# SKA-INAF/caesar-mrcnn

Measured on AMD Instinct MI355X. Metric: train images/sec (whole node) + detect ms/image, ResNet-101 256x256, higher is better.
Workload: dtype f32; 1 GPU; resnet101+FPN 256x256 3-class (+bg), nimg_per_gpu=4, train step (fwd+bwd+SGD), 512 train ROIs, 2000 proposals; global_batch=4, parallelism=dp1, weights=random init (Keras defaults)

## Files before the change

caesar-mrcnn_amd/_hip.py:

```python
import ctypes as C
import os
import threading

PKG_DIR = os.path.dirname(os.path.abspath(__file__))
LIB_PATH = os.path.join(PKG_DIR, "libmrcnn_hip.so")


class HipPathError(RuntimeError):
    pass


class ConvDesc(C.Structure):
    _fields_ = [(n, C.c_int32) for n in (
        "N", "H", "W", "Cin", "Cout", "KH", "KW", "stride", "pad_t", "pad_l", "OH", "OW",
        "act", "res_mode", "out_mode", "cmod")] + [
        ("out_n_stride", C.c_int64), ("out_h_stride", C.c_int64), ("out_w_stride", C.c_int64)]


class ConvProblem(C.Structure):
    _fields_ = [("d", ConvDesc)] + [(n, C.c_void_p) for n in ("x", "w", "bias", "scale", "shift", "res", "out", "z_out")]


class WgradProblem(C.Structure):
    _fields_ = [("d", ConvDesc), ("x", C.c_void_p), ("dy", C.c_void_p), ("dw", C.c_void_p), ("accumulate", C.c_int32)]
# ... 120 lines not shown
    "mrcnn_conv2d_fwd_h16_res": (C.c_int, [C.POINTER(ConvDesc), C.c_int] + [_P] * 9),
    "mrcnn_conv2d_fwd_h16_supported": (C.c_int, [C.POINTER(ConvDesc), C.c_int]),
    "mrcnn_conv2d_dgrad_ep_h16": (C.c_int, [C.POINTER(ConvDesc), C.c_int, _P, _P, _P, _P, C.POINTER(BwdEpilogueH16), _P]),
    "mrcnn_conv2d_dgrad_ep": (C.c_int, [C.POINTER(ConvDesc), _P, _P, _P, _P, C.POINTER(BwdEpilogue), _P, C.c_size_t, _P]),
    "mrcnn_conv2d_wgrad_h16_workspace": (C.c_size_t, [C.POINTER(ConvDesc)]),
    "mrcnn_conv2d_wgrad_h16": (C.c_int, [C.POINTER(ConvDesc), C.c_int, _P, _P, _P, _P, C.c_size_t, C.c_int, C.c_float, _P]),
    "mrcnn_mask_out_fwd_h16": (C.c_int, [C.c_int, _P, _P, _P, _P, C.c_int64, C.c_int, C.c_int, _P]),
    "mrcnn_mask_out_bwd_h16": (C.c_int, [C.c_int] + [_P] * 8 + [C.c_int64, C.c_int, C.c_int, C.c_int, C.c_int, C.c_float, _P]),
    "mrcnn_weights_to_h16": (C.c_int, [_P, _P, _P, C.c_int, C.c_int, C.c_int, C.c_int, C.c_int, _P]),
    "mrcnn_weights_to_h16_batched": (C.c_int, [_P, _P, C.c_int, C.c_int, C.c_int, _P]),
    "mrcnn_cast_to_h16": (C.c_int, [_P, _P, C.c_int64, C.c_int, C.c_float, _P]),
    "mrcnn_epilogue_bwd_h16": (C.c_int, [C.c_int] + [_P] * 10 + [C.c_int64, C.c_int, C.c_int, C.c_float, _P]),
    "mrcnn_epilogue_bwd_h16_dy": (C.c_int, [C.c_int] + [_P] * 11 + [C.c_int64, C.c_int, C.c_int, C.c_float, _P]),
    "mrcnn_cast_from_h16": (C.c_int, [_P, _P, C.c_int64, C.c_int, C.c_float, _P]),
    "mrcnn_axpy_from_h16": (C.c_int, [_P, _P, C.c_int64, C.c_int, C.c_float, _P]),
    "mrcnn_rpn_targets_workspace": (C.c_size_t, [C.POINTER(RpnTargetDesc)]),
    "mrcnn_rpn_targets": (C.c_int, [C.POINTER(RpnTargetDesc)] + [_P] * 7 + [C.c_size_t, _P]),
    "mrcnn_detection_workspace": (C.c_size_t, [C.POINTER(DetectionDesc)]),
    "mrcnn_detection_fwd": (C.c_int, [C.POINTER(DetectionDesc)] + [_P] * 6 + [C.c_size_t, _P]),
    "mrcnn_losses_workspace": (C.c_size_t, [C.POINTER(LossDesc)]),
    "mrcnn_losses_fwd_bwd": (C.c_int, [C.POINTER(LossDesc)] + [_P] * 18 + [C.c_size_t, _P]),
    "mrcnn_grad_prepare": (C.c_int, [_P, _P, C.c_float, _P, C.c_int64, _P, _P]),
    "mrcnn_sumsq": (C.c_int, [_P, C.c_int64, _P, _P]),
    "mrcnn_sgd_momentum": (C.c_int, [_P, _P, _P, _P, C.c_float, C.c_float, C.c_float, _P, C.c_int64, _P]),
    "mrcnn_sgd_momentum_guarded": (C.c_int, [_P, _P, _P, _P, C.c_float, C.c_float, C.c_float, _P, C.c_int64, _P, _P]),
    "mrcnn_winograd_buffer_floats": (C.c_size_t, [C.c_int, C.c_int, C.c_int, C.c_int, C.c_int]),
    "mrcnn_winograd_weights": (C.c_int, [_P, _P, C.c_int, C.c_int, C.c_int, _P]),
    "mrcnn_gemm_batched_f32": (C.c_int, [_P, _P, _P, C.c_int, C.c_int, C.c_int, C.c_int, _P]),
    "mrcnn_winograd_gemm": (C.c_int, [_P, _P, _P, C.c_int, C.c_int, C.c_int, C.c_int, _P]),
    "mrcnn_winograd_group_floats": (C.c_size_t, [C.POINTER(WinoGroup), C.c_int, C.c_int]),
    "mrcnn_winograd_input_g": (C.c_int, [_P, _P, C.c_int, C.c_int, C.c_int, C.c_int, C.POINTER(WinoGroup), _P]),
    "mrcnn_winograd_weights_g": (C.c_int, [_P, _P, C.c_int, C.c_int, C.c_int, C.c_int, _P]),
    "mrcnn_winograd_output_g": (C.c_int, [_P, _P, _P, _P, _P, _P, C.c_int, C.c_int, C.c_int, C.c_int, C.c_int, C.POINTER(WinoGroup), _P]),
    "mrcnn_winograd_output_bwd_g": (C.c_int, [_P, _P, _P, _P, _P, _P, _P, _P, _P, _P, C.c_int, C.c_int, C.c_int, C.c_int, C.c_int,
                                             C.POINTER(WinoGroup), _P]),
    "mrcnn_winograd_output_bwd_zmask_g": (C.c_int, [_P] * 10 + [C.c_int, C.c_int, C.c_int, C.c_int, C.POINTER(WinoGroup), _P]),
    "mrcnn_winograd_dy_g": (C.c_int, [_P, _P, C.c_int, C.c_int, C.c_int, C.c_int, C.POINTER(WinoGroup), _P]),
    "mrcnn_winograd_dw_g": (C.c_int, [_P, _P, C.c_int, C.c_int, C.c_int, C.c_int, C.c_int, _P]),
    "mrcnn_deconv2x2_gemm": (C.c_int, [_P, _P, _P, _P, C.c_int, C.c_int, C.c_int, C.c_int, C.c_int, C.c_int, _P]),
    "mrcnn_allreduce_load": (C.c_int, [C.c_char_p]),
    "mrcnn_allreduce_unique_id": (C.c_int, [_P]),
    "mrcnn_allreduce_init": (C.c_int, [C.POINTER(_P), _P, C.c_int, C.c_int]),
    "mrcnn_allreduce_scratch": (C.c_size_t, [C.c_int, C.c_int64, C.c_int]),
    "mrcnn_allreduce_grad": (C.c_int, [_P, _P, C.c_int64, C.c_int64, C.c_int, _P, C.c_size_t, _P]),
    "mrcnn_allreduce_direct_plan": (C.c_int, [C.c_int, C.c_int, C.c_int64, C.c_int64, C.c_int, _P, _P, _P, _P]),
    "mrcnn_allreduce_direct_simulate": (C.c_int, [_P, _P, C.c_size_t, C.c_int, C.c_int64, C.c_int64, _P]),
    "mrcnn_allreduce_destroy": (C.c_int, [_P]),
    "mrcnn_allreduce_last_error": (C.c_char_p, []),
    "mrcnn_tuning_set": (C.c_int, [C.c_char_p, C.c_longlong]),
    "mrcnn_hip_version": (C.c_char_p, []),
}

_lib = None
_proxy = None
_tape = None
_tape_owner = None

_NO_RECORD = ("_workspace", "_tiles_check", "_outline_check", "_draw_check", "_supported", "_status_offset", "_version", "mrcnn_allreduce_", "_scratch", "_floats")


class _LibProxy(object):

    def __init__(self, real):
        self._real = real

    def __getattr__(self, name):
        real = getattr(self._real, name)
        if any(k in name for k in _NO_RECORD):
            f = real
        else:
            def f(*args, _real=real):
                rc = _real(*args)
                t = _tape
                if t is not None and not rc and _tape_owner == threading.get_ident():
                    t.append((_real, args))
                return rc
        setattr(self, name, f)
        return f


def tape_begin():
    global _tape, _tape_owner
    assert _tape is None, "a launch tape is already being recorded"
    _tape, _tape_owner = [], threading.get_ident()
    return _tape


def tape_end():
    global _tape, _tape_owner
    t, _tape, _tape_owner = _tape, None, None
    return t
# ... 83 lines not shown
```

caesar-mrcnn_amd/csrc/winograd.hip:

```cpp
#include "common.h"
#include <type_traits>
#include <string.h>

template <int CV> struct WinoVec;
template <> struct WinoVec<4> { typedef f32x4 type; };
template <> struct WinoVec<2> { typedef float type __attribute__((ext_vector_type(2))); };

template <int OT, typename V> __device__ __forceinline__ void wino_bt(const V (&d)[OT + 2], V (&t)[OT + 2]) {
    if constexpr (OT == 2) {
        t[0] = d[0] - d[2];
        t[1] = d[1] + d[2];
        t[2] = d[2] - d[1];
        t[3] = d[1] - d[3];
    } else {
        const V a = d[4] - 4.f * d[2], b = d[3] - 4.f * d[1], c = d[4] - d[2], e = 2.f * (d[3] - d[1]);
        t[0] = 4.f * d[0] - 5.f * d[2] + d[4];
        t[1] = a + b;
        t[2] = a - b;
        t[3] = c + e;
        t[4] = c - e;
        t[5] = 4.f * d[1] - 5.f * d[3] + d[5];
    }
}
template <int OT, typename V> __device__ __forceinline__ void wino_at(const V (&m)[OT + 2], V (&y)[OT]) {
// ... 158 lines not shown
            vec zv, o;
#pragma unroll
            for (int e = 0; e < CV; ++e) {
                zv[e] = y[b][e] + bi[e];
                float v = sc[e] * zv[e] + sh[e];
                if (act == MRCNN_ACT_RELU) v = fmaxf(v, 0.f);
                o[e] = v;
            }
            if (z) *(vec*)(z + addr) = zv;
            *(vec*)(out + addr) = o;
        }
    }
}

template <int OTH, int OTW, int CV>
__global__ __launch_bounds__(256) void winograd_output_kernel(const float* __restrict__ Mt, float* __restrict__ out, float* __restrict__ z,
                                                              const float* __restrict__ bias, const float* __restrict__ scale,
                                                              const float* __restrict__ shift, int N, int H, int W, int C, long long T,
                                                              long long Tp, int act, const WinoGrp g) {
    typedef typename WinoVec<CV>::type vec;
    const int cn = C / CV;
    const long long i = (long long)blockIdx.x * 256 + threadIdx.x;
    if (i >= T * cn) return;
    const long long t = i / cn;
    const int c = (int)(i - t * cn) * CV;
    vec bi = {}, sc, sh = {};
#pragma unroll
    for (int e = 0; e < CV; ++e) sc[e] = 1.f;
    if (bias) bi = *(const vec*)(bias + c);
    if (scale) { sc = *(const vec*)(scale + c); sh = *(const vec*)(shift + c); }
    wino_output_tile<OTH, OTW, CV>(Mt, out, z, bi, sc, sh, H, W, C, Tp, act, g, t, c);
}

template <int OTH, int OTW, int CV>
__device__ __forceinline__ void wino_output_bwd_tile(const float* __restrict__ Mt, float* __restrict__ dz_out, const float* __restrict__ below_out,
                                                     const float* __restrict__ below_z, const typename WinoVec<CV>::type sc,
                                                     const typename WinoVec<CV>::type mu, const typename WinoVec<CV>::type rs,
                                                     const typename WinoVec<CV>::type fsh, bool zmask, bool want_dg, int H, int W, int C,
                                                     long long Tp, int act, const WinoGrp& g, long long t, int c,
                                                     typename WinoVec<CV>::type& a_db, typename WinoVec<CV>::type& a_dg,
                                                     typename WinoVec<CV>::type& a_bias) {
    typedef typename WinoVec<CV>::type vec;
    constexpr int ITH = OTH + 2, ITW = OTW + 2;
    const WinoTile q = wino_tile(t, g.th_n, g.tw_n);
    vec s[OTH][ITW];
#pragma unroll
    for (int k = 0; k < ITW; ++k) {
        vec col[ITH], o[OTH];
#pragma unroll
        for (int r = 0; r < ITH; ++r) col[r] = *(const vec*)(Mt + ((long long)(r * ITW + k) * Tp + t) * C + c);
        wino_at<OTH>(col, o);
#pragma unroll
        for (int a = 0; a < OTH; ++a) s[a][k] = o[a];
    }
#pragma unroll
    for (int a = 0; a < OTH; ++a) {
        vec y[OTW];
        wino_at<OTW>(s[a], y);
        const int oh = g.oh0 + OTH * q.th + a;
        if (oh >= H) continue;
#pragma unroll
        for (int b = 0; b < OTW; ++b) {
            const int ow = g.ow0 + OTW * q.tw + b;
            if (ow >= W) continue;
            const long long addr = (((long long)q.n * H + oh) * W + ow) * C + c;
            vec gg = y[b], dz, zz = {};
            if (want_dg || zmask) zz = *(const vec*)(below_z + addr);
            if (act == MRCNN_ACT_RELU) {
                if (zmask) {
#pragma unroll
                    for (int e = 0; e < CV; ++e) {
                        const float v = sc[e] * zz[e] + fsh[e];
                        gg[e] = v > 0.f ? gg[e] : 0.f;
                    }
                } else {
                    const vec oo = *(const vec*)(below_out + addr);
#pragma unroll
                    for (int e = 0; e < CV; ++e) gg[e] = oo[e] > 0.f ? gg[e] : 0.f;
                }
            }
#pragma unroll
            for (int e = 0; e < CV; ++e) dz[e] = gg[e] * sc[e];
            *(vec*)(dz_out + addr) = dz;
            if (want_dg) {
#pragma unroll
                for (int e = 0; e < CV; ++e) a_dg[e] += gg[e] * (zz[e] - mu[e]) * rs[e];
            }
#pragma unroll
            for (int e = 0; e < CV; ++e) { a_db[e] += gg[e]; a_bias[e] += dz[e]; }
        }
    }
}

template <int OTH, int OTW, int CV>
__global__ __launch_bounds__(256) void winograd_output_bwd_kernel(const float* __restrict__ Mt, float* __restrict__ dz_out,
                                                                  const float* __restrict__ below_out, const float* __restrict__ below_z,
                                                                  const float* __restrict__ scale, const float* __restrict__ mean,
                                                                  const float* __restrict__ rstd, float* dgamma, float* dbeta, float* dbias,
                                                                  int N, int H, int W, int C, long long T, long long Tp, int act,
                                                                  long long tiles_per_block, int lg, const WinoGrp g,
                                                                  const float* __restrict__ fwd_shift) {
    typedef typename WinoVec<CV>::type vec;
    constexpr int ITH = OTH + 2, ITW = OTW + 2;
    __shared__ float sacc[3 * 4 * 256];
    const int L = 1 << lg, R = 256 >> lg;
    for (int c = threadIdx.x; c < 3 * CV * L; c += 256) sacc[c] = 0.f;
    __syncthreads();
    const int rsub = threadIdx.x >> lg, lane = threadIdx.x & (L - 1);
    const int c = lane * CV;
    const long long t0 = (long long)blockIdx.x * tiles_per_block;
    long long t1 = t0 + tiles_per_block;
    if (t1 > T) t1 = T;
    vec sc, mu = {}, rs = {}, fsh = {};
#pragma unroll
    for (int e = 0; e < CV; ++e) sc[e] = 1.f;
    if (scale) sc = *(const vec*)(scale + c);
    if (dgamma) { mu = *(const vec*)(mean + c); rs = *(const vec*)(rstd + c); }
    const bool zmask = fwd_shift != nullptr;
    if (zmask) fsh = *(const vec*)(fwd_shift + c);
    vec a_db = {}, a_dg = {}, a_bias = {};
    for (long long t = t0 + rsub; t < t1; t += R)
        wino_output_bwd_tile<OTH, OTW, CV>(Mt, dz_out, below_out, below_z, sc, mu, rs, fsh, zmask, dgamma != nullptr, H, W, C, Tp, act, g, t, c,
                                           a_db, a_dg, a_bias);
#pragma unroll
    for (int k = 0; k < CV; ++k) {
        if (dbeta || dgamma) atomicAdd(&sacc[lane * CV + k], a_db[k]);
        if (dgamma) atomicAdd(&sacc[CV * L + lane * CV + k], a_dg[k]);
        if (dbias) atomicAdd(&sacc[2 * CV * L + lane * CV + k], a_bias[k]);
    }
    __syncthreads();
    for (int j = threadIdx.x; j < CV * L; j += 256) {
        if (dbeta) atomicAdd(&dbeta[j], sacc[j]);
        if (dgamma) atomicAdd(&dgamma[j], sacc[CV * L + j]);
        if (dbias) atomicAdd(&dbias[j], sacc[2 * CV * L + j]);
    }
}

template <int OTH, int OTW, int CV>
__global__ __launch_bounds__(256) void winograd_dy_kernel(const float* __restrict__ dy, float* __restrict__ dM, int N, int H, int W, int C,
                                                          long long T, long long Tp, const WinoGrp g) {
    typedef typename WinoVec<CV>::type vec;
    constexpr int ITH = OTH + 2, ITW = OTW + 2;
    const int cn = C / CV;
    const long long i = (long long)blockIdx.x * 256 + threadIdx.x;
    if (i >= T * cn) return;
    const long long t = i / cn;
    const int c = (int)(i - t * cn) * CV;
    const WinoTile q = wino_tile(t, g.th_n, g.tw_n);
    vec u[ITH][OTW];
#pragma unroll
    for (int b = 0; b < OTW; ++b) {
        vec col[OTH], o[ITH];
#pragma unroll
        for (int a = 0; a < OTH; ++a) {
            const int oh = g.oh0 + OTH * q.th + a, ow = g.ow0 + OTW * q.tw + b;
            vec val = {};
            if (oh < H && ow < W) val = *(const vec*)(dy + (((long long)q.n * H + oh) * W + ow) * C + c);
            col[a] = val;
        }
        wino_a<OTH>(col, o);
#pragma unroll
        for (int r = 0; r < ITH; ++r) u[r][b] = o[r];
    }
#pragma unroll
    for (int r = 0; r < ITH; ++r) {
        vec m[ITW];
        wino_a<OTW>(u[r], m);
// ... 211 lines not shown

extern "C" size_t mrcnn_winograd_group_floats(const mrcnn_wino_group* g, int N, int C) {
    if (!g || N <= 0 || C <= 0 || (g->oth != 2 && g->oth != 4) || (g->otw != 2 && g->otw != 4) || g->th_n <= 0 || g->tw_n <= 0) return 0;
    return (size_t)wino_grp_nb(g) * (size_t)wino_rows(wino_grp_tiles(g, N)) * (size_t)C;
}

extern "C" int mrcnn_winograd_input_g(const float* x, float* V, int N, int H, int W, int C, const mrcnn_wino_group* g, void* stream) {
    if (!x || !V || !wino_grp_ok(g, N, H, W, C)) return MRCNN_ERR_ARG;
    const long long T = wino_grp_tiles(g, N);
    const WinoGrp k = {g->th_n, g->tw_n, g->oh0, g->ow0};
    const dim3 g4((unsigned)cdiv64(T * C / 4, 256)), g2((unsigned)cdiv64(T * C / 2, 256));
    WINO_LAUNCH_G(winograd_input_kernel, g, g4, g2, x, V, N, H, W, C, T, wino_rows(T), k);
    return mrcnn_launch_status();
}

extern "C" int mrcnn_winograd_weights_g(const float* w, float* U, int Cin, int Cout, int oth, int otw, void* stream) {
    if (!w || !U || Cin <= 0 || Cout <= 0 || (oth != 2 && oth != 4) || (otw != 2 && otw != 4)) return MRCNN_ERR_ARG;
    const dim3 grid((unsigned)cdiv64((long long)Cin * Cout, 256));
    WINO_LAUNCH_W(winograd_weight_kernel, oth, otw, grid, w, U, Cin, Cout);
    return mrcnn_launch_status();
}

extern "C" int mrcnn_winograd_output_g(const float* Mt, float* out, float* z, const float* bias, const float* scale, const float* shift,
                                       int N, int H, int W, int C, int act, const mrcnn_wino_group* g, void* stream) {
    if (!Mt || !out || !wino_grp_ok(g, N, H, W, C) || (scale && !shift)) return MRCNN_ERR_ARG;
    if (act != MRCNN_ACT_NONE && act != MRCNN_ACT_RELU) return MRCNN_ERR_UNSUPPORTED;
    const long long T = wino_grp_tiles(g, N);
    const WinoGrp k = {g->th_n, g->tw_n, g->oh0, g->ow0};
    const dim3 g4((unsigned)cdiv64(T * C / 4, 256)), g2((unsigned)cdiv64(T * C / 2, 256));
    WINO_LAUNCH_G(winograd_output_kernel, g, g4, g2, Mt, out, z, bias, scale, shift, N, H, W, C, T, wino_rows(T), act, k);
    return mrcnn_launch_status();
}

static int wino_output_bwd_g(const float* Mt, float* dz_below, const float* below_out, const float* below_z, const float* scale,
                             const float* mean, const float* rstd, float* dgamma, float* dbeta, float* dbias, int N, int H,
                             int W, int C, int act, const mrcnn_wino_group* g, void* stream, const float* fwd_shift);

extern "C" int mrcnn_winograd_output_bwd_g(const float* Mt, float* dz_below, const float* below_out, const float* below_z, const float* scale,
                                           const float* mean, const float* rstd, float* dgamma, float* dbeta, float* dbias, int N, int H,
                                           int W, int C, int act, const mrcnn_wino_group* g, void* stream) {
    return wino_output_bwd_g(Mt, dz_below, below_out, below_z, scale, mean, rstd, dgamma, dbeta, dbias, N, H, W, C, act, g, stream, nullptr);
}

extern "C" int mrcnn_winograd_output_bwd_zmask_g(const float* Mt, float* dz_below, const float* below_z, const float* scale,
                                                 const float* shift, const float* mean, const float* rstd, float* dgamma, float* dbeta,
                                                 float* dbias, int N, int H, int W, int C, const mrcnn_wino_group* g, void* stream) {
    if (!below_z || !scale || !shift) return MRCNN_ERR_ARG;
    return wino_output_bwd_g(Mt, dz_below, nullptr, below_z, scale, mean, rstd, dgamma, dbeta, dbias, N, H, W, C, MRCNN_ACT_RELU, g, stream, shift);
}

static int wino_output_bwd_g(const float* Mt, float* dz_below, const float* below_out, const float* below_z, const float* scale,
                             const float* mean, const float* rstd, float* dgamma, float* dbeta, float* dbias, int N, int H,
                             int W, int C, int act, const mrcnn_wino_group* g, void* stream, const float* fwd_shift) {
    if (!Mt || !dz_below || !wino_grp_ok(g, N, H, W, C)) return MRCNN_ERR_ARG;
    if ((act != MRCNN_ACT_NONE && act != MRCNN_ACT_RELU) || (act == MRCNN_ACT_RELU && !below_out && !fwd_shift)) return MRCNN_ERR_ARG;
    if (dgamma && (!below_z || !mean || !rstd)) return MRCNN_ERR_ARG;
    const int cv = wino_grp_cv(g);
    const int cn = C / cv;
    if (cn > 256 || (cn & (cn - 1))) return MRCNN_ERR_UNSUPPORTED;
    int lg = 0;
    while ((1 << lg) < cn) ++lg;
    const long long T = wino_grp_tiles(g, N);
    const long long R = 256 >> lg;
    long long per = (T + 2047) / 2048;
    per = (per + R - 1) / R * R;
    const dim3 grid((unsigned)cdiv64(T, per));
    const WinoGrp k = {g->th_n, g->tw_n, g->oh0, g->ow0};
    WINO_LAUNCH_G(winograd_output_bwd_kernel, g, grid, grid, Mt, dz_below, below_out, below_z, scale, mean, rstd, dgamma, dbeta, dbias, N, H, W,
                  C, T, wino_rows(T), act, per, lg, k, fwd_shift);
    return mrcnn_launch_status();
}

extern "C" int mrcnn_winograd_dy_g(const float* dy, float* dM, int N, int H, int W, int C, const mrcnn_wino_group* g, void* stream) {
    if (!dy || !dM || !wino_grp_ok(g, N, H, W, C)) return MRCNN_ERR_ARG;
    const long long T = wino_grp_tiles(g, N);
    const WinoGrp k = {g->th_n, g->tw_n, g->oh0, g->ow0};
    const dim3 g4((unsigned)cdiv64(T * C / 4, 256)), g2((unsigned)cdiv64(T * C / 2, 256));
    WINO_LAUNCH_G(winograd_dy_kernel, g, g4, g2, dy, dM, N, H, W, C, T, wino_rows(T), k);
    return mrcnn_launch_status();
}

extern "C" int mrcnn_winograd_dw_g(const float* dU, float* dw_hwio, int Cin, int Cout, int accumulate, int oth, int otw, void* stream) {
    if (!dU || !dw_hwio || Cin <= 0 || Cout <= 0 || (oth != 2 && oth != 4) || (otw != 2 && otw != 4)) return MRCNN_ERR_ARG;
    const dim3 grid((unsigned)cdiv64((long long)Cin * Cout, 256));
    WINO_LAUNCH_W(winograd_dw_kernel, oth, otw, grid, dU, dw_hwio, Cin, Cout, accumulate);
    return mrcnn_launch_status();
}

extern "C" size_t mrcnn_winograd_buffer_floats(int N, int H, int W, int C, int tile) {
    if ((tile != 2 && tile != 4) || (tile == 2 && ((H & 1) || (W & 1)))) return 0;
    if (!(N > 0 && H > 0 && W > 0 && C > 0 && !(C & 3))) return 0;
    const mrcnn_wino_group g = {tile, tile, wino_tdim(H, tile), wino_tdim(W, tile), 0, 0};
    return mrcnn_winograd_group_floats(&g, N, C);
}

extern "C" int mrcnn_winograd_weights(const float* w, float* U, int Cin, int Cout, int tile, void* stream) {
    return mrcnn_winograd_weights_g(w, U, Cin, Cout, tile, tile, stream);
}

extern "C" int mrcnn_winograd_gemm(const float* V, const float* U, float* Mt, int nb, int rows, int K, int N, void* stream) {
    if (!V || !U || !Mt || nb <= 0 || rows <= 0 || rows % 128 || K <= 0 || K % 16 || N <= 0 || N % 128) return MRCNN_ERR_ARG;
    const long long M = (long long)nb * rows;
// ... 41 lines not shown
```

caesar-mrcnn_amd/ops.py:

```python
import ctypes as C
import math
import os

import torch

from . import _hip
from ._hip import (ACT_NONE, ACT_RELU, ACT_SIGMOID, OUT_DECONV2, OUT_NHWC, RES_NONE, RES_SAME, RES_UP2,
                   check, current_stream, ptr)

BN_EPS = 1e-3


def _need_cuda(*ts):
    for t in ts:
        if t is not None and not t.is_cuda:
            raise _hip.HipPathError("hot-path operators need device tensors (got a CPU tensor)")
        if t is not None and not t.is_contiguous():
            raise _hip.HipPathError("hot-path operators need contiguous tensors")


def same_padding(size, k, stride):
    out = -(-size // stride)
    total = max((out - 1) * stride + k - size, 0)
    return out, total // 2
# ... 1243 lines not shown


def winograd_v_floats(xshape, tile=None):
    N, H, W, Cin = xshape
    if tile is None:
        tile = winograd_tile(xshape)
    lib = _hip.lib()
    return sum(lib.mrcnn_winograd_group_floats(C.byref(g), N, Cin) for g in winograd_groups(H, W, tile))


def conv2d_winograd(x, U, bias=None, scale=None, shift=None, act=ACT_NONE, out=None, z_out=None, keep_v=None, after_input=None):
    _need_cuda(x, bias, scale, shift, out, z_out, keep_v)
    N, H, W, _ = x.shape
    cout = (U[0] if isinstance(U, (list, tuple)) else U).shape[2]
    if out is None:
        out = empty((N, H, W, cout), torch.float32, x.device)
    lib = _hip.lib()

    def finish(g, Mt):
        check(lib.mrcnn_winograd_output_g(ptr(Mt), ptr(out), ptr(z_out), ptr(bias), ptr(scale), ptr(shift), N, H, W, cout, act, C.byref(g),
                                          current_stream()), "mrcnn_winograd_output_g")

    _winograd_run(x, U, finish, keep_v, after_input)
    return out


def conv2d_dgrad_ep_winograd(dz, Ut, below_out, below_z, scale, mean, rstd, dgamma, dbeta, dbias, act, fwd_shift=None):
    _need_cuda(dz, below_out, below_z, scale, mean, rstd, dgamma, dbeta, dbias, fwd_shift)
    N, H, W, _ = dz.shape
    cout = (Ut[0] if isinstance(Ut, (list, tuple)) else Ut).shape[2]
    out = empty((N, H, W, cout), torch.float32, dz.device)
    lib = _hip.lib()
    zmask = act == ACT_RELU and fwd_shift is not None and below_z is not None and scale is not None

    def finish(g, Mt):
        if zmask:
            check(lib.mrcnn_winograd_output_bwd_zmask_g(ptr(Mt), ptr(out), ptr(below_z), ptr(scale), ptr(fwd_shift), ptr(mean), ptr(rstd),
                                                        ptr(dgamma), ptr(dbeta), ptr(dbias), N, H, W, cout, C.byref(g), current_stream()),
                  "mrcnn_winograd_output_bwd_zmask_g")
            return
        check(lib.mrcnn_winograd_output_bwd_g(ptr(Mt), ptr(out), ptr(below_out), ptr(below_z), ptr(scale), ptr(mean), ptr(rstd),
                                              ptr(dgamma), ptr(dbeta), ptr(dbias), N, H, W, cout, act, C.byref(g), current_stream()),
              "mrcnn_winograd_output_bwd_g")

    _winograd_run(dz, Ut, finish)
    return out


def conv2d_wgrad_winograd(V, xshape, dz, dw, accumulate=False, tile=None):
    _need_cuda(V, dz, dw)
    N, H, W, Cin = xshape
    cout = dz.shape[3]
    if tile is None:
        tile = winograd_tile(xshape)
    groups = winograd_groups(H, W, tile)
    lib = _hip.lib()
    nvs = [lib.mrcnn_winograd_group_floats(C.byref(g), N, Cin) for g in groups]
    nms = [lib.mrcnn_winograd_group_floats(C.byref(g), N, cout) for g in groups]
    assert V.numel() == sum(nvs), "V was made with another tiling"
    dM_all = workspace(max(nms) * 4, dz.device, "winograd_dm")
    dU_all = workspace(36 * Cin * cout * 4, dz.device, "winograd_du")
    off = 0
    for gi, g in enumerate(groups):
        nb = _wino_nb(g)
        rows = nms[gi] // (nb * cout)
        T = N * g.th_n * g.tw_n
        dM = dM_all[:nms[gi] * 4].view(torch.float32).view(nb, rows, cout)
        dU = dU_all[:nb * Cin * cout * 4].view(torch.float32).view(nb, Cin, cout)
        check(lib.mrcnn_winograd_dy_g(ptr(dz), ptr(dM), N, H, W, cout, C.byref(g), current_stream()), "mrcnn_winograd_dy_g")
        Vv = V[off:off + nvs[gi]].view(nb, rows, Cin)
        off += nvs[gi]
        items = [(Vv[k, :T].view(T, 1, 1, Cin), dM[k, :T].view(T, 1, 1, cout), (1, 1, Cin, cout), 1, "valid", dU[k].view(1, 1, Cin, cout), False)
                 for k in range(nb)]
        per = 16 if nb == 16 else 12
        for i in range(0, nb, per):
            if not conv2d_wgrad_multi(items[i:i + per]):
                for x_, dy_, wshape, stride, padding, dw_, acc in items[i:i + per]:
                    conv2d_wgrad(x_, dy_, wshape, stride, padding, dw=dw_, accumulate=acc)
# ... 150 lines not shown
```

include/mrcnn_hip.h:

```cpp
#ifndef MRCNN_HIP_H
#define MRCNN_HIP_H

#include <stddef.h>
#include <stdint.h>

#ifdef __cplusplus
extern "C" {
#endif

#define MRCNN_OK 0
#define MRCNN_ERR_ARG (-1)
#define MRCNN_ERR_LAUNCH (-2)
#define MRCNN_ERR_WORKSPACE (-3)
#define MRCNN_ERR_UNSUPPORTED (-4)

#define MRCNN_ACT_NONE 0
#define MRCNN_ACT_RELU 1
#define MRCNN_ACT_SIGMOID 2

#define MRCNN_RES_NONE 0
#define MRCNN_RES_SAME 1
#define MRCNN_RES_UP2 2

#define MRCNN_OUT_NHWC 0
// ... 293 lines not shown
int mrcnn_losses_fwd_bwd(const mrcnn_loss_desc* d, const int32_t* rpn_match, const float* rpn_bbox_t,
                         const float* rpn_class_logits, const float* rpn_bbox,
                         const int32_t* target_class_ids, const float* target_bbox,
                         const float* target_mask, const int32_t* active_class_ids,
                         const float* mrcnn_class_logits, const float* mrcnn_bbox,
                         const float* mrcnn_mask, float* losses, float* d_rpn_class_logits,
                         float* d_rpn_bbox, float* d_mrcnn_class_logits, float* d_mrcnn_bbox,
                         float* d_mrcnn_mask, void* workspace, size_t workspace_bytes, void* stream);

int mrcnn_grad_prepare(float* grads, const float* params, float grad_scale, const float* gran_coef,
                       int64_t n, float* sumsq_out, void* stream);
int mrcnn_sumsq(const float* g, int64_t n, float* out_scalar, void* stream);
int mrcnn_sgd_momentum(float* params, float* momentum_buf, const float* grads, const float* sumsq,
                       float clipnorm, float lr, float momentum, const float* gran_coef, int64_t n,
                       void* stream);
int mrcnn_sgd_momentum_guarded(float* params, float* momentum_buf, const float* grads, const float* sumsq,
                               float clipnorm, float lr, float momentum, const float* gran_coef, int64_t n,
                               unsigned* skipped_steps, void* stream);

typedef struct mrcnn_wino_group {
    int oth, otw;
    int th_n, tw_n;
    int oh0, ow0;
} mrcnn_wino_group;
size_t mrcnn_winograd_group_floats(const mrcnn_wino_group* g, int N, int C);
size_t mrcnn_winograd_buffer_floats(int N, int H, int W, int C, int tile);
int mrcnn_winograd_weights(const float* w_hwio, float* U, int Cin, int Cout, int tile, void* stream);
int mrcnn_winograd_weights_g(const float* w_hwio, float* U, int Cin, int Cout, int oth, int otw, void* stream);
int mrcnn_winograd_input_g(const float* x, float* V, int N, int H, int W, int C, const mrcnn_wino_group* g, void* stream);
int mrcnn_gemm_batched_f32(const float* V, const float* U, float* Mt, int nb, int rows, int K, int Cout, void* stream);
int mrcnn_winograd_gemm(const float* V, const float* U, float* Mt, int nb, int rows, int K, int Cout, void* stream);
int mrcnn_winograd_output_g(const float* Mt, float* out, float* z_out, const float* bias, const float* scale, const float* shift,
                            int N, int H, int W, int C, int act, const mrcnn_wino_group* g, void* stream);
int mrcnn_winograd_output_bwd_g(const float* Mt, float* dz_below, const float* below_out, const float* below_z, const float* scale,
                                const float* mean, const float* rstd, float* dgamma, float* dbeta, float* dbias, int N, int H, int W,
                                int C, int act, const mrcnn_wino_group* g, void* stream);
int mrcnn_winograd_output_bwd_zmask_g(const float* Mt, float* dz_below, const float* below_z, const float* scale, const float* shift,
                                      const float* mean, const float* rstd, float* dgamma, float* dbeta, float* dbias, int N, int H,
                                      int W, int C, const mrcnn_wino_group* g, void* stream);
int mrcnn_winograd_dy_g(const float* dy, float* dM, int N, int H, int W, int C, const mrcnn_wino_group* g, void* stream);
int mrcnn_winograd_dw_g(const float* dU, float* dw_hwio, int Cin, int Cout, int accumulate, int oth, int otw, void* stream);

int mrcnn_deconv2x2_gemm(const float* x, const float* w_gemm, const float* bias, float* out, int N, int H, int W, int Cin, int Cd,
                         int act, void* stream);

#define MRCNN_UNIQUE_ID_BYTES 128
#define MRCNN_ALLREDUCE_RCCL 0
#define MRCNN_ALLREDUCE_DIRECT 1
int mrcnn_allreduce_load(const char* librccl_path);
int mrcnn_allreduce_unique_id(void* id_128_bytes);
int mrcnn_allreduce_init(void** comm, const void* id_128_bytes, int rank, int world);
size_t mrcnn_allreduce_scratch(int world, int64_t max_range_floats, int algo);
int mrcnn_allreduce_grad(void* comm, float* grads, int64_t start, int64_t end, int algo, float* scratch,
                         size_t scratch_bytes, void* stream);
int mrcnn_allreduce_direct_plan(int world, int rank, int64_t start, int64_t end, int phase, int64_t* plan, int64_t* own_off,
                                int64_t* own_len, int64_t* slot_stride);
int mrcnn_allreduce_direct_simulate(float* const* grads, float* const* scratch, size_t scratch_bytes, int world, int64_t start,
                                    int64_t end, void* stream);
int mrcnn_allreduce_destroy(void* comm);
const char* mrcnn_allreduce_last_error(void);

int mrcnn_tuning_set(const char* key, long long value);

const char* mrcnn_hip_version(void);

#ifdef __cplusplus
}
#endif
#endif
```

Baseline: 111.7 images/s.

## Replace atomic reductions in Winograd output backward with per-block partials and sum kernel

The Winograd data-gradient output kernel now runs as a persistent grid capped at four blocks per CU. Each block writes per-channel partial sums for dbeta, dgamma and dbias to a workspace, and a separate kernel reduces them, replacing the shared and global atomics. The kernel also issues all Mt tile loads up front through buffer loads with 32-bit offsets, uses fast division for tile indexing, and is templated on the mask mode. This trades atomic contention and 64-bit address math for an extra kernel launch, a workspace, and higher register pressure from the preloaded tiles.

After: 113.1 images/s, median of 6. +1.3%, better.

```diff
diff --git a/caesar-mrcnn_amd/_hip.py b/caesar-mrcnn_amd/_hip.py
--- a/caesar-mrcnn_amd/_hip.py
+++ b/caesar-mrcnn_amd/_hip.py
@@ -176,9 +176,10 @@
     "mrcnn_winograd_input_g": (C.c_int, [_P, _P, C.c_int, C.c_int, C.c_int, C.c_int, C.POINTER(WinoGroup), _P]),
     "mrcnn_winograd_weights_g": (C.c_int, [_P, _P, C.c_int, C.c_int, C.c_int, C.c_int, _P]),
     "mrcnn_winograd_output_g": (C.c_int, [_P, _P, _P, _P, _P, _P, C.c_int, C.c_int, C.c_int, C.c_int, C.c_int, C.POINTER(WinoGroup), _P]),
-    "mrcnn_winograd_output_bwd_g": (C.c_int, [_P, _P, _P, _P, _P, _P, _P, _P, _P, _P, C.c_int, C.c_int, C.c_int, C.c_int, C.c_int,
-                                             C.POINTER(WinoGroup), _P]),
-    "mrcnn_winograd_output_bwd_zmask_g": (C.c_int, [_P] * 10 + [C.c_int, C.c_int, C.c_int, C.c_int, C.POINTER(WinoGroup), _P]),
+    "mrcnn_winograd_output_bwd_rows": (C.c_int, [C.POINTER(WinoGroup), C.c_int, C.c_int]),
+    "mrcnn_winograd_output_bwd_g": (C.c_int, [_P] * 8 + [C.c_int, C.c_int, C.c_int, C.c_int, C.c_int, C.POINTER(WinoGroup), _P]),
+    "mrcnn_winograd_output_bwd_zmask_g": (C.c_int, [_P] * 8 + [C.c_int, C.c_int, C.c_int, C.c_int, C.POINTER(WinoGroup), _P]),
+    "mrcnn_winograd_output_bwd_sums": (C.c_int, [_P, C.c_int, C.c_int, _P, _P, _P, _P]),
     "mrcnn_winograd_dy_g": (C.c_int, [_P, _P, C.c_int, C.c_int, C.c_int, C.c_int, C.POINTER(WinoGroup), _P]),
     "mrcnn_winograd_dw_g": (C.c_int, [_P, _P, C.c_int, C.c_int, C.c_int, C.c_int, C.c_int, _P]),
     "mrcnn_deconv2x2_gemm": (C.c_int, [_P, _P, _P, _P, C.c_int, C.c_int, C.c_int, C.c_int, C.c_int, C.c_int, _P]),
@@ -200,7 +201,7 @@
 _tape = None
 _tape_owner = None
 
-_NO_RECORD = ("_workspace", "_tiles_check", "_outline_check", "_draw_check", "_supported", "_status_offset", "_version", "mrcnn_allreduce_", "_scratch", "_floats")
+_NO_RECORD = ("_workspace", "_tiles_check", "_outline_check", "_draw_check", "_supported", "_status_offset", "_version", "mrcnn_allreduce_", "_scratch", "_floats", "_bwd_rows")
 
 
 class _LibProxy(object):
diff --git a/caesar-mrcnn_amd/csrc/winograd.hip b/caesar-mrcnn_amd/csrc/winograd.hip
--- a/caesar-mrcnn_amd/csrc/winograd.hip
+++ b/caesar-mrcnn_amd/csrc/winograd.hip
@@ -214,107 +214,157 @@
     wino_output_tile<OTH, OTW, CV>(Mt, out, z, bi, sc, sh, H, W, C, Tp, act, g, t, c);
 }
 
-template <int OTH, int OTW, int CV>
-__device__ __forceinline__ void wino_output_bwd_tile(const float* __restrict__ Mt, float* __restrict__ dz_out, const float* __restrict__ below_out,
-                                                     const float* __restrict__ below_z, const typename WinoVec<CV>::type sc,
-                                                     const typename WinoVec<CV>::type mu, const typename WinoVec<CV>::type rs,
-                                                     const typename WinoVec<CV>::type fsh, bool zmask, bool want_dg, int H, int W, int C,
-                                                     long long Tp, int act, const WinoGrp& g, long long t, int c,
-                                                     typename WinoVec<CV>::type& a_db, typename WinoVec<CV>::type& a_dg,
-                                                     typename WinoVec<CV>::type& a_bias) {
-    typedef typename WinoVec<CV>::type vec;
-    constexpr int ITH = OTH + 2, ITW = OTW + 2;
-    const WinoTile q = wino_tile(t, g.th_n, g.tw_n);
-    vec s[OTH][ITW];
-#pragma unroll
-    for (int k = 0; k < ITW; ++k) {
-        vec col[ITH], o[OTH];
-#pragma unroll
-        for (int r = 0; r < ITH; ++r) col[r] = *(const vec*)(Mt + ((long long)(r * ITW + k) * Tp + t) * C + c);
-        wino_at<OTH>(col, o);
-#pragma unroll
-        for (int a = 0; a < OTH; ++a) s[a][k] = o[a];
-    }
-#pragma unroll
-    for (int a = 0; a < OTH; ++a) {
-        vec y[OTW];
-        wino_at<OTW>(s[a], y);
-        const int oh = g.oh0 + OTH * q.th + a;
-        if (oh >= H) continue;
-#pragma unroll
-        for (int b = 0; b < OTW; ++b) {
-            const int ow = g.ow0 + OTW * q.tw + b;
-            if (ow >= W) continue;
-            const long long addr = (((long long)q.n * H + oh) * W + ow) * C + c;
-            vec gg = y[b], dz, zz = {};
-            if (want_dg || zmask) zz = *(const vec*)(below_z + addr);
-            if (act == MRCNN_ACT_RELU) {
-                if (zmask) {
-#pragma unroll
-                    for (int e = 0; e < CV; ++e) {
-                        const float v = sc[e] * zz[e] + fsh[e];
-                        gg[e] = v > 0.f ? gg[e] : 0.f;
-                    }
-                } else {
-                    const vec oo = *(const vec*)(below_out + addr);
-#pragma unroll
-                    for (int e = 0; e < CV; ++e) gg[e] = oo[e] > 0.f ? gg[e] : 0.f;
-                }
-            }
-#pragma unroll
-            for (int e = 0; e < CV; ++e) dz[e] = gg[e] * sc[e];
-            *(vec*)(dz_out + addr) = dz;
-            if (want_dg) {
-#pragma unroll
-                for (int e = 0; e < CV; ++e) a_dg[e] += gg[e] * (zz[e] - mu[e]) * rs[e];
-            }
-#pragma unroll
-            for (int e = 0; e < CV; ++e) { a_db[e] += gg[e]; a_bias[e] += dz[e]; }
-        }
-    }
-}
-
-template <int OTH, int OTW, int CV>
+template <int CV>
+__device__ __forceinline__ typename WinoVec<CV>::type wino_buffer_load(__amdgpu_buffer_rsrc_t rsrc, unsigned voff, unsigned soff) {
+    typename WinoVec<CV>::type r;
+    if constexpr (CV == 2) {
+        const auto v = __builtin_amdgcn_raw_buffer_load_b64(rsrc, (int)voff, (int)soff, 0);
+        r[0] = __uint_as_float(v[0]); r[1] = __uint_as_float(v[1]);
+    } else {
+        const auto v = __builtin_amdgcn_raw_buffer_load_b128(rsrc, (int)voff, (int)soff, 0);
+        r[0] = __uint_as_float(v[0]); r[1] = __uint_as_float(v[1]); r[2] = __uint_as_float(v[2]); r[3] = __uint_as_float(v[3]);
+    }
+    return r;
+}
+
+template <int OTH, int OTW, int CV, int MASK>
 __global__ __launch_bounds__(256) void winograd_output_bwd_kernel(const float* __restrict__ Mt, float* __restrict__ dz_out,
                                                                   const float* __restrict__ below_out, const float* __restrict__ below_z,
                                                                   const float* __restrict__ scale, const float* __restrict__ mean,
-                                                                  const float* __restrict__ rstd, float* dgamma, float* dbeta, float* dbias,
-                                                                  int N, int H, int W, int C, long long T, long long Tp, int act,
-                                                                  long long tiles_per_block, int lg, const WinoGrp g,
-                                                                  const float* __restrict__ fwd_shift) {
+                                                                  const float* __restrict__ rstd, const float* __restrict__ fwd_shift,
+                                                                  float* __restrict__ partials, int want_dg, int H, int W, int C, unsigned T,
+                                                                  long long Tp, int lg, const WinoGrp g, const FastDiv d_th,
+                                                                  const FastDiv d_tw) {
     typedef typename WinoVec<CV>::type vec;
     constexpr int ITH = OTH + 2, ITW = OTW + 2;
     __shared__ float sacc[3 * 4 * 256];
     const int L = 1 << lg, R = 256 >> lg;
-    for (int c = threadIdx.x; c < 3 * CV * L; c += 256) sacc[c] = 0.f;
-    __syncthreads();
     const int rsub = threadIdx.x >> lg, lane = threadIdx.x & (L - 1);
     const int c = lane * CV;
-    const long long t0 = (long long)blockIdx.x * tiles_per_block;
-    long long t1 = t0 + tiles_per_block;
-    if (t1 > T) t1 = T;
     vec sc, mu = {}, rs = {}, fsh = {};
 #pragma unroll
     for (int e = 0; e < CV; ++e) sc[e] = 1.f;
     if (scale) sc = *(const vec*)(scale + c);
-    if (dgamma) { mu = *(const vec*)(mean + c); rs = *(const vec*)(rstd + c); }
-    const bool zmask = fwd_shift != nullptr;
-    if (zmask) fsh = *(const vec*)(fwd_shift + c);
+    if (want_dg) { mu = *(const vec*)(mean + c); rs = *(const vec*)(rstd + c); }
+    if (MASK == 1) fsh = *(const vec*)(fwd_shift + c);
+    const bool need_z = MASK == 1 || want_dg;
     vec a_db = {}, a_dg = {}, a_bias = {};
-    for (long long t = t0 + rsub; t < t1; t += R)
-        wino_output_bwd_tile<OTH, OTW, CV>(Mt, dz_out, below_out, below_z, sc, mu, rs, fsh, zmask, dgamma != nullptr, H, W, C, Tp, act, g, t, c,
-                                           a_db, a_dg, a_bias);
-#pragma unroll
-    for (int k = 0; k < CV; ++k) {
-        if (dbeta || dgamma) atomicAdd(&sacc[lane * CV + k], a_db[k]);
-        if (dgamma) atomicAdd(&sacc[CV * L + lane * CV + k], a_dg[k]);
-        if (dbias) atomicAdd(&sacc[2 * CV * L + lane * CV + k], a_bias[k]);
+    const unsigned step = gridDim.x * (unsigned)R;
+    const __amdgpu_buffer_rsrc_t rsrc_m = __builtin_amdgcn_make_buffer_rsrc((void*)Mt, 0, 0xFFFFFFF0u, 0x00020000);
+    const unsigned mstride = (unsigned)Tp * (unsigned)C * 4u;
+    for (unsigned t = blockIdx.x * (unsigned)R + rsub; t < T; t += step) {
+        const unsigned q = fast_div(t, d_tw), n = fast_div(q, d_th);
+        const int tw = (int)(t - q * (unsigned)g.tw_n), th = (int)(q - n * (unsigned)g.th_n);
+        const int oh0 = g.oh0 + OTH * th, ow0 = g.ow0 + OTW * tw;
+        vec m[ITH][ITW], zz[OTH][OTW], oo[OTH][OTW];
+        const unsigned moff = (t * (unsigned)C + c) * 4u;
+#pragma unroll
+        for (int r = 0; r < ITH; ++r)
+#pragma unroll
+            for (int k = 0; k < ITW; ++k)
+                m[r][k] = wino_buffer_load<CV>(rsrc_m, moff, (unsigned)(r * ITW + k) * mstride);
+        const unsigned base = (((n * (unsigned)H + oh0) * W + ow0) * C + c) * 4u;
+        unsigned roff[OTH], coff[OTW];
+#pragma unroll
+        for (int a = 0; a < OTH; ++a) roff[a] = base + (unsigned)(min(a, H - 1 - oh0) * W * C) * 4u;
+#pragma unroll
+        for (int b = 0; b < OTW; ++b) coff[b] = (unsigned)(min(b, W - 1 - ow0) * C) * 4u;
+        if (need_z) {
+#pragma unroll
+            for (int a = 0; a < OTH; ++a)
+#pragma unroll
+                for (int b = 0; b < OTW; ++b) zz[a][b] = *(const vec*)((const char*)below_z + (roff[a] + coff[b]));
+        } else {
+#pragma unroll
+            for (int a = 0; a < OTH; ++a)
+#pragma unroll
+                for (int b = 0; b < OTW; ++b) zz[a][b] = vec{};
+        }
+        if (MASK == 2) {
+#pragma unroll
+            for (int a = 0; a < OTH; ++a)
+#pragma unroll
+                for (int b = 0; b < OTW; ++b) oo[a][b] = *(const vec*)((const char*)below_out + (roff[a] + coff[b]));
+        }
+        vec s[OTH][ITW];
+#pragma unroll
+        for (int k = 0; k < ITW; ++k) {
+            vec col[ITH], o[OTH];
+#pragma unroll
+            for (int r = 0; r < ITH; ++r) col[r] = m[r][k];
+            wino_at<OTH>(col, o);
+#pragma unroll
+            for (int a = 0; a < OTH; ++a) s[a][k] = o[a];
+        }
+#pragma unroll
+        for (int a = 0; a < OTH; ++a) {
+            vec y[OTW];
+            wino_at<OTW>(s[a], y);
+#pragma unroll
+            for (int b = 0; b < OTW; ++b) {
+                const bool inside = oh0 + a < H && ow0 + b < W;
+                vec gg = y[b], dz;
+                if (MASK == 1) {
+#pragma unroll
+                    for (int e = 0; e < CV; ++e) {
+                        const float v = sc[e] * zz[a][b][e] + fsh[e];
+                        gg[e] = v > 0.f ? gg[e] : 0.f;
+                    }
+                } else if (MASK == 2) {
+#pragma unroll
+                    for (int e = 0; e < CV; ++e) gg[e] = oo[a][b][e] > 0.f ? gg[e] : 0.f;
+                }
+#pragma unroll
+                for (int e = 0; e < CV; ++e) {
+                    gg[e] = inside ? gg[e] : 0.f;
+                    dz[e] = gg[e] * sc[e];
+                }
+                if (inside) *(vec*)((char*)dz_out + (roff[a] + coff[b])) = dz;
+                if (want_dg) {
+#pragma unroll
+                    for (int e = 0; e < CV; ++e) a_dg[e] += gg[e] * (zz[a][b][e] - mu[e]) * rs[e];
+                }
+#pragma unroll
+                for (int e = 0; e < CV; ++e) { a_db[e] += gg[e]; a_bias[e] += dz[e]; }
+            }
+        }
+    }
+    if (!partials) return;
+#pragma unroll
+    for (int e = 0; e < CV; ++e) {
+        sacc[(0 * R + rsub) * C + c + e] = a_db[e];
+        sacc[(1 * R + rsub) * C + c + e] = a_dg[e];
+        sacc[(2 * R + rsub) * C + c + e] = a_bias[e];
     }
     __syncthreads();
-    for (int j = threadIdx.x; j < CV * L; j += 256) {
-        if (dbeta) atomicAdd(&dbeta[j], sacc[j]);
-        if (dgamma) atomicAdd(&dgamma[j], sacc[CV * L + j]);
-        if (dbias) atomicAdd(&dbias[j], sacc[2 * CV * L + j]);
+    for (int j = threadIdx.x; j < 3 * C; j += 256) {
+        const int k = j / C, cc = j - k * C;
+        float v = sacc[k * R * C + cc];
+        for (int r = 1; r < R; ++r) v += sacc[(k * R + r) * C + cc];
+        partials[(long long)blockIdx.x * 3 * C + j] = v;
+    }
+}
+
+#define WINO_SUMS_COLS 16
+#define WINO_SUMS_SLICES 64
+__global__ __launch_bounds__(WINO_SUMS_COLS * WINO_SUMS_SLICES) void winograd_bwd_sums_kernel(const float* __restrict__ partials, int rows,
+                                                                                              int C, float* dgamma, float* dbeta,
+                                                                                              float* dbias) {
+    __shared__ float sm[WINO_SUMS_SLICES][WINO_SUMS_COLS];
+    const int col = threadIdx.x % WINO_SUMS_COLS, slice = threadIdx.x / WINO_SUMS_COLS;
+    const int j = blockIdx.x * WINO_SUMS_COLS + col;
+    const int k = j / C;
+    float* dst = k == 0 ? dbeta : k == 1 ? dgamma : k == 2 ? dbias : nullptr;
+    float v = 0.f;
+    if (dst) {
+#pragma unroll 8
+        for (int r = slice; r < rows; r += WINO_SUMS_SLICES) v += partials[(long long)r * 3 * C + j];
+    }
+    sm[slice][col] = v;
+    __syncthreads();
+    if (slice == 0 && dst) {
+        for (int s = 1; s < WINO_SUMS_SLICES; ++s) v += sm[s][col];
+        atomicAdd(&dst[j - k * C], v);
     }
 }
 
@@ -592,42 +642,69 @@
     return mrcnn_launch_status();
 }
 
-static int wino_output_bwd_g(const float* Mt, float* dz_below, const float* below_out, const float* below_z, const float* scale,
-                             const float* mean, const float* rstd, float* dgamma, float* dbeta, float* dbias, int N, int H,
-                             int W, int C, int act, const mrcnn_wino_group* g, void* stream, const float* fwd_shift);
-
-extern "C" int mrcnn_winograd_output_bwd_g(const float* Mt, float* dz_below, const float* below_out, const float* below_z, const float* scale,
-                                           const float* mean, const float* rstd, float* dgamma, float* dbeta, float* dbias, int N, int H,
-                                           int W, int C, int act, const mrcnn_wino_group* g, void* stream) {
-    return wino_output_bwd_g(Mt, dz_below, below_out, below_z, scale, mean, rstd, dgamma, dbeta, dbias, N, H, W, C, act, g, stream, nullptr);
-}
-
-extern "C" int mrcnn_winograd_output_bwd_zmask_g(const float* Mt, float* dz_below, const float* below_z, const float* scale,
-                                                 const float* shift, const float* mean, const float* rstd, float* dgamma, float* dbeta,
-                                                 float* dbias, int N, int H, int W, int C, const mrcnn_wino_group* g, void* stream) {
-    if (!below_z || !scale || !shift) return MRCNN_ERR_ARG;
-    return wino_output_bwd_g(Mt, dz_below, nullptr, below_z, scale, mean, rstd, dgamma, dbeta, dbias, N, H, W, C, MRCNN_ACT_RELU, g, stream, shift);
-}
-
-static int wino_output_bwd_g(const float* Mt, float* dz_below, const float* below_out, const float* below_z, const float* scale,
-                             const float* mean, const float* rstd, float* dgamma, float* dbeta, float* dbias, int N, int H,
-                             int W, int C, int act, const mrcnn_wino_group* g, void* stream, const float* fwd_shift) {
-    if (!Mt || !dz_below || !wino_grp_ok(g, N, H, W, C)) return MRCNN_ERR_ARG;
-    if ((act != MRCNN_ACT_NONE && act != MRCNN_ACT_RELU) || (act == MRCNN_ACT_RELU && !below_out && !fwd_shift)) return MRCNN_ERR_ARG;
-    if (dgamma && (!below_z || !mean || !rstd)) return MRCNN_ERR_ARG;
-    const int cv = wino_grp_cv(g);
-    const int cn = C / cv;
-    if (cn > 256 || (cn & (cn - 1))) return MRCNN_ERR_UNSUPPORTED;
+static int wino_bwd_lanes_lg(const mrcnn_wino_group* g, int C) {
+    const int cn = C / wino_grp_cv(g);
+    if (cn <= 0 || cn > 256 || (cn & (cn - 1)) || cn * wino_grp_cv(g) != C) return -1;
     int lg = 0;
     while ((1 << lg) < cn) ++lg;
+    return lg;
+}
+extern "C" int mrcnn_winograd_output_bwd_rows(const mrcnn_wino_group* g, int N, int C) {
+    if (!g || N <= 0 || (g->oth != 2 && g->oth != 4) || (g->otw != 2 && g->otw != 4) || g->th_n <= 0 || g->tw_n <= 0) return 0;
+    const int lg = wino_bwd_lanes_lg(g, C);
+    if (lg < 0) return 0;
+    const long long T = wino_grp_tiles(g, N), R = 256 >> lg, cap = 4LL * mrcnn_num_cus();
+    const long long wgs = cdiv64(T, R);
+    return (int)(wgs < cap ? wgs : cap);
+}
+
+template <int MASK>
+static int wino_output_bwd_launch(const float* Mt, float* dz_below, const float* below_out, const float* below_z, const float* scale,
+                                  const float* mean, const float* rstd, const float* fwd_shift, float* partials, int N, int H, int W,
+                                  int C, const mrcnn_wino_group* g, void* stream) {
+    const int lg = wino_bwd_lanes_lg(g, C);
     const long long T = wino_grp_tiles(g, N);
-    const long long R = 256 >> lg;
-    long long per = (T + 2047) / 2048;
-    per = (per + R - 1) / R * R;
-    const dim3 grid((unsigned)cdiv64(T, per));
+    if (lg < 0) return MRCNN_ERR_UNSUPPORTED;
+    if ((long long)wino_grp_nb(g) * wino_rows(T) * C * 4 >= (1LL << 32) || (long long)N * H * W * C * 4 >= (1LL << 32)) return MRCNN_ERR_UNSUPPORTED;
+    const dim3 grid((unsigned)mrcnn_winograd_output_bwd_rows(g, N, C));
     const WinoGrp k = {g->th_n, g->tw_n, g->oh0, g->ow0};
-    WINO_LAUNCH_G(winograd_output_bwd_kernel, g, grid, grid, Mt, dz_below, below_out, below_z, scale, mean, rstd, dgamma, dbeta, dbias, N, H, W,
-                  C, T, wino_rows(T), act, per, lg, k, fwd_shift);
+    const int want_dg = partials && mean && rstd && below_z;
+#define WINO_BWD_INST(oth, otw, cv)                                                                                            \
+    hipLaunchKernelGGL((winograd_output_bwd_kernel<oth, otw, cv, MASK>), grid, dim3(256), 0, (hipStream_t)stream, Mt, dz_below, below_out, \
+                       below_z, scale, mean, rstd, fwd_shift, partials, want_dg, H, W, C, (unsigned)T, wino_rows(T), lg, k,    \
+                       make_fastdiv((unsigned)g->th_n), make_fastdiv((unsigned)g->tw_n))
+    if (g->oth == 2 && g->otw == 2) WINO_BWD_INST(2, 2, 4);
+    else if (g->oth == 4 && g->otw == 4) WINO_BWD_INST(4, 4, 2);
+    else if (g->oth == 4) WINO_BWD_INST(4, 2, 2);
+    else WINO_BWD_INST(2, 4, 2);
+#undef WINO_BWD_INST
+    return mrcnn_launch_status();
+}
+
+extern "C" int mrcnn_winograd_output_bwd_g(const float* Mt, float* dz_below, const float* below_out, const float* below_z, const float* scale,
+                                           const float* mean, const float* rstd, float* partials, int N, int H, int W, int C, int act,
+                                           const mrcnn_wino_group* g, void* stream) {
+    if (!Mt || !dz_below || !wino_grp_ok(g, N, H, W, C) || (!mean != !rstd) || (mean && !below_z)) return MRCNN_ERR_ARG;
+    if (act == MRCNN_ACT_NONE)
+        return wino_output_bwd_launch<0>(Mt, dz_below, nullptr, below_z, scale, mean, rstd, nullptr, partials, N, H, W, C, g, stream);
+    if (act != MRCNN_ACT_RELU || !below_out) return MRCNN_ERR_ARG;
+    return wino_output_bwd_launch<2>(Mt, dz_below, below_out, below_z, scale, mean, rstd, nullptr, partials, N, H, W, C, g, stream);
+}
+
+extern "C" int mrcnn_winograd_output_bwd_zmask_g(const float* Mt, float* dz_below, const float* below_z, const float* scale,
+                                                 const float* shift, const float* mean, const float* rstd, float* partials, int N, int H,
+                                                 int W, int C, const mrcnn_wino_group* g, void* stream) {
+    if (!Mt || !dz_below || !wino_grp_ok(g, N, H, W, C) || !below_z || !scale || !shift || (!mean != !rstd)) return MRCNN_ERR_ARG;
+    return wino_output_bwd_launch<1>(Mt, dz_below, nullptr, below_z, scale, mean, rstd, shift, partials, N, H, W, C, g, stream);
+}
+
+extern "C" int mrcnn_winograd_output_bwd_sums(const float* partials, int rows, int C, float* dgamma, float* dbeta, float* dbias,
+                                              void* stream) {
+    if (!partials || rows <= 0 || C <= 0) return MRCNN_ERR_ARG;
+    if (!dgamma && !dbeta && !dbias) return MRCNN_OK;
+    const dim3 grid((unsigned)cdiv64(3LL * C, WINO_SUMS_COLS));
+    hipLaunchKernelGGL(winograd_bwd_sums_kernel, grid, dim3(WINO_SUMS_COLS * WINO_SUMS_SLICES), 0, (hipStream_t)stream, partials, rows, C,
+                       dgamma, dbeta, dbias);
     return mrcnn_launch_status();
 }
 
diff --git a/caesar-mrcnn_amd/ops.py b/caesar-mrcnn_amd/ops.py
--- a/caesar-mrcnn_amd/ops.py
+++ b/caesar-mrcnn_amd/ops.py
@@ -1299,18 +1299,32 @@
     out = empty((N, H, W, cout), torch.float32, dz.device)
     lib = _hip.lib()
     zmask = act == ACT_RELU and fwd_shift is not None and below_z is not None and scale is not None
+    if dgamma is None:
+        mean = rstd = None
+    want_sums = dgamma is not None or dbeta is not None or dbias is not None
+    rows = [lib.mrcnn_winograd_output_bwd_rows(C.byref(g), N, cout) for g in winograd_groups(H, W, _wino_tile_of(Ut))]
+    assert min(rows) > 0, "channel count does not fit the Winograd data-gradient transform"
+    part = ptr(workspace(sum(rows) * 3 * cout * 4, dz.device, "winograd_bwd_sums")) if want_sums else None
+    done = []
 
     def finish(g, Mt):
+        p = None
+        if want_sums:
+            p = part + sum(done) * 3 * cout * 4
+            done.append(rows[len(done)])
         if zmask:
             check(lib.mrcnn_winograd_output_bwd_zmask_g(ptr(Mt), ptr(out), ptr(below_z), ptr(scale), ptr(fwd_shift), ptr(mean), ptr(rstd),
-                                                        ptr(dgamma), ptr(dbeta), ptr(dbias), N, H, W, cout, C.byref(g), current_stream()),
+                                                        p, N, H, W, cout, C.byref(g), current_stream()),
                   "mrcnn_winograd_output_bwd_zmask_g")
             return
         check(lib.mrcnn_winograd_output_bwd_g(ptr(Mt), ptr(out), ptr(below_out), ptr(below_z), ptr(scale), ptr(mean), ptr(rstd),
-                                              ptr(dgamma), ptr(dbeta), ptr(dbias), N, H, W, cout, act, C.byref(g), current_stream()),
+                                              p, N, H, W, cout, act, C.byref(g), current_stream()),
               "mrcnn_winograd_output_bwd_g")
 
     _winograd_run(dz, Ut, finish)
+    if want_sums:
+        check(lib.mrcnn_winograd_output_bwd_sums(part, sum(done), cout, ptr(dgamma), ptr(dbeta), ptr(dbias), current_stream()),
+              "mrcnn_winograd_output_bwd_sums")
     return out
 
 
diff --git a/include/mrcnn_hip.h b/include/mrcnn_hip.h
--- a/include/mrcnn_hip.h
+++ b/include/mrcnn_hip.h
@@ -349,12 +349,14 @@
 int mrcnn_winograd_gemm(const float* V, const float* U, float* Mt, int nb, int rows, int K, int Cout, void* stream);
 int mrcnn_winograd_output_g(const float* Mt, float* out, float* z_out, const float* bias, const float* scale, const float* shift,
                             int N, int H, int W, int C, int act, const mrcnn_wino_group* g, void* stream);
+int mrcnn_winograd_output_bwd_rows(const mrcnn_wino_group* g, int N, int C);
 int mrcnn_winograd_output_bwd_g(const float* Mt, float* dz_below, const float* below_out, const float* below_z, const float* scale,
-                                const float* mean, const float* rstd, float* dgamma, float* dbeta, float* dbias, int N, int H, int W,
-                                int C, int act, const mrcnn_wino_group* g, void* stream);
+                                const float* mean, const float* rstd, float* partials, int N, int H, int W, int C, int act,
+                                const mrcnn_wino_group* g, void* stream);
 int mrcnn_winograd_output_bwd_zmask_g(const float* Mt, float* dz_below, const float* below_z, const float* scale, const float* shift,
-                                      const float* mean, const float* rstd, float* dgamma, float* dbeta, float* dbias, int N, int H,
-                                      int W, int C, const mrcnn_wino_group* g, void* stream);
+                                      const float* mean, const float* rstd, float* partials, int N, int H, int W, int C,
+                                      const mrcnn_wino_group* g, void* stream);
+int mrcnn_winograd_output_bwd_sums(const float* partials, int rows, int C, float* dgamma, float* dbeta, float* dbias, void* stream);
 int mrcnn_winograd_dy_g(const float* dy, float* dM, int N, int H, int W, int C, const mrcnn_wino_group* g, void* stream);
 int mrcnn_winograd_dw_g(const float* dU, float* dw_hwio, int Cin, int Cout, int accumulate, int oth, int otw, void* stream);
 
```
